# chongminggao/CIRS-codes

Hardware: AMD Instinct MI355X
Metric: simulator env-steps/s (collect + PPO update in the timed region), KuaishouEnv (higher is better)
Workload: dtype f32 (policy/tracker; rollout on the fp32 MFMA, PPO head products fp32-accurate from two fp16 pieces per operand (3 f16 MFMAs per product), fp32 accumulate) + f64 (env rewards, GAE)

## Files before the change

### cirs-codes_amd/csrc/ppo.hip

```cpp
#include "internal.h"
#include "bf16x6.h"
#include "small_gemm.h"
#include "permutation.h"
#include "policy_kernels.h"

namespace cirs {
typedef float f32x4 __attribute__((ext_vector_type(4)));


constexpr int kBwdWaves = 4;
__host__ __device__ inline int n_row_blocks_of(int n_pad) { return (n_pad / kTileM + kBwdWaves - 1) / kBwdWaves; }
__host__ __device__ inline size_t dwa_slab_stride(int I) { return (((size_t)I * 64 + I) + 3) & ~(size_t)3; }
__host__ __device__ inline int n_dwa_slabs_of(int n_pad) { return n_row_blocks_of(n_pad); }

struct PpoLayout {
    long w1, b1, w2, b2, wa, ba, wc, bc, total, trunk;
};
__host__ __device__ inline PpoLayout ppo_layout(int I, int S) {
    PpoLayout L;
    L.w1 = 0; L.b1 = L.w1 + (long)kH * S; L.w2 = L.b1 + kH; L.b2 = L.w2 + (long)kH * kH;
    L.trunk = L.b2 + kH;
    L.wa = L.trunk; L.ba = L.wa + (long)I * kH; L.wc = L.ba + I; L.bc = L.wc + kH; L.total = L.bc + 1;
    return L;
}
// ... 144 lines not shown
__global__ __launch_bounds__(1024) void prepare_tail_kernel(cirs_ppo_cfg cfg, cirs_traj traj, cirs_ppo_batch out, const double* __restrict__ unnorm_ret,
                                                            double* __restrict__ rms_state, const int32_t* __restrict__ n_dev, int B, int S, int n_compact,
                                                            PermKeys keys, int n_perm, long perm_upper, int32_t* __restrict__ perm_out) {
    __shared__ double red[1024];
    __shared__ double s_mean;
    const int N = *n_dev;
    const int b = blockIdx.x;
    if (b == 0) { returns_block(cfg, unnorm_ret, N, rms_state, out.ret, red, s_mean); return; }
    if (b <= n_compact) { compact_obs_elem(traj, out, (long)(b - 1) * 1024 + threadIdx.x, N, B, S); return; }
    const long g = (long)(b - 1 - n_compact) * 1024 + threadIdx.x;
    const int c = (int)(g / perm_upper);
    const long i = g - (long)c * perm_upper;
    if (c < n_perm && i < N) perm_out[(size_t)c * N + i] = (int32_t)permute_index(i, N, perm_half_bits((uint64_t)N), perm_key_of(keys, c));
}

typedef Planes2 HPl;
constexpr float kScWa = 256.f, kScH2 = 64.f;
#define HPL_SET(P, H, L) do { (P).h = __builtin_bit_cast(f16x8, H); (P).l = __builtin_bit_cast(f16x8, L); } while (0)
#define hsplit8 split8h
#define hmfma_split2 mfma_f16x3_split2
#define hmfma_pair mfma_f16x3_pair
constexpr float kScZ = kScWa * kScH2, kScZi = 1.0f / kScZ;
constexpr int kPlaneTileU4 = 1536;
struct MbView {
    float *obs, *adv, *ret, *v_s, *logp_old;
    int32_t* act;
    float *h1, *h2, *value;
    float *lse, *ez, *za;
    float *c_logp, *c_ent, *h_ent, *dvalue;
    float *ent_row;
    float *clip_row, *vf_row;
    long *dst_row;
    float *da2, *da1;
    float *dh2p;
    float *entp;
    float *dwap;
    float *red;
    float *normp;
    float *dwp;
    uint4 *wa_planes;
    uint4 *h2z, *h2b;
    int *sync;
    void* head_ws;
};

constexpr int kSyncInts = 288, kSyncA0 = 256;
__device__ __forceinline__ void flag_arrive(int* flags, int b) {
    if (threadIdx.x == 0) __hip_atomic_store(flags + b, 1, __ATOMIC_RELAXED, __HIP_MEMORY_SCOPE_AGENT);
}
__device__ int g_handoff_lost = 0;
__device__ __forceinline__ void flags_wait(const int* flags, int n) {
    int spins = 0;
    for (;;) {
        int mine = 1;
        for (int q = threadIdx.x; q < n; q += blockDim.x) mine &= __hip_atomic_load(flags + q, __ATOMIC_RELAXED, __HIP_MEMORY_SCOPE_AGENT) != 0;
        if (__syncthreads_and(mine)) break;
        if (++spins >= (1 << 20)) {
            if (threadIdx.x == 0) atomicAdd(&g_handoff_lost, 1);
            break;
        }
        __builtin_amdgcn_s_sleep(1);
    }
}
__global__ void handoff_status_kernel(int* __restrict__ out, int reset) {
    out[0] = g_handoff_lost;
// ... 13 lines not shown
__host__ __device__ inline int snap_floats(int S) { return kH * (S + 66) + kH + 1; }
__host__ __device__ inline int snap_stride(int S) { return (snap_floats(S) + 3) & ~3; }
__host__ inline size_t dwp_floats(int n_pad, int S) {
    const size_t a = (size_t)(n_pad / kTileM) * (kH * (kH + 1) + kH * (S + 1) + (kH + 1)) + 64, b = (size_t)(n_pad / 8) * snap_stride(S) + 64;
    return a > b ? a : b;
}
__host__ inline size_t mb_ws_floats(int n_pad, int I, int S) {
    const size_t nch = n_chunks_of(I);
    size_t f = 0;
    f += (size_t)n_pad * S + 4 * (size_t)n_pad;
    f += n_pad;
    f += 2 * (size_t)n_pad * kH + n_pad;
    f += 3 * (size_t)n_pad;
    f += 4 * (size_t)n_pad + n_pad;
    f += 2 * (size_t)n_pad + 2 * (size_t)n_pad + 8;
    f += 2 * (size_t)n_pad * kH;
    f += nch * (size_t)n_pad * kH + nch * (size_t)n_pad;
    f += (size_t)n_dwa_slabs_of(n_pad) * dwa_slab_stride(I);
    f += kSyncInts + 4;
    f += 64 + 1024;
    f += dwp_floats(n_pad, S);
    f += (size_t)cdiv(I, kTileN) * kPlaneTileU4 * 4;
    f += 2 * (size_t)n_pad * 96;
    f += (size_t)n_pad * kH + 4 * nch * (size_t)n_pad;
    return f;
}

__host__ inline MbView carve(void* ws, int n_pad, int I, int S) {
    float* p = (float*)ws;
    const size_t nch = n_chunks_of(I);
    MbView v;
    auto take = [&](size_t n) { float* r = p; p += (n + 3) & ~(size_t)3; return r; };
    v.obs = take((size_t)n_pad * S); v.adv = take(n_pad); v.ret = take(n_pad); v.v_s = take(n_pad); v.logp_old = take(n_pad);
    v.act = (int32_t*)take(n_pad);
    v.h1 = take((size_t)n_pad * kH); v.h2 = take((size_t)n_pad * kH); v.value = take(n_pad);
    v.lse = take(n_pad); v.ez = take(n_pad); v.za = take(n_pad);
    v.c_logp = take(n_pad); v.c_ent = take(n_pad); v.h_ent = take(n_pad); v.dvalue = take(n_pad); v.ent_row = take(n_pad);
    v.clip_row = take(n_pad); v.vf_row = take(n_pad);
    v.dst_row = (long*)take(2 * (size_t)n_pad + 4);
    v.da2 = take((size_t)n_pad * kH); v.da1 = take((size_t)n_pad * kH);
    v.dh2p = take(nch * (size_t)n_pad * kH); v.entp = take(nch * (size_t)n_pad);
    v.dwap = take((size_t)n_dwa_slabs_of(n_pad) * dwa_slab_stride(I));
    v.sync = (int*)take(kSyncInts);
    v.red = take(64);
    v.normp = take(1024);
    v.dwp = take(dwp_floats(n_pad, S));
    v.wa_planes = (uint4*)take((size_t)cdiv(I, kTileN) * kPlaneTileU4 * 4);
    v.h2z = (uint4*)take((size_t)n_pad * 96); v.h2b = (uint4*)take((size_t)n_pad * 96);
    v.head_ws = (void*)p;
    return v;
}

__device__ __forceinline__ void adv_stats_block(const float* __restrict__ adv_flat, const int32_t* __restrict__ idx, int m,
                                                int enable, float* __restrict__ red, float* sh ) {
    __shared__ float s_mean;
    const int tid = threadIdx.x;
    if (!enable) {
        if (tid == 0) { red[0] = 0.f; red[1] = 1.f; }
        return;
    }
    float acc = 0.f;
    for (int i = tid; i < m; i += 256) acc += adv_flat[idx[i]];
    sh[tid] = acc;
    __syncthreads();
    for (int s = 128; s > 0; s >>= 1) {
        if (tid < s) sh[tid] += sh[tid + s];
        __syncthreads();
    }
    if (tid == 0) s_mean = sh[0] / (float)m;
    __syncthreads();
    const float mean = s_mean;
// ... 259 lines not shown

constexpr int kTStride = 36;
constexpr int kRSize = kTileN * kH + 2 * kTileN;
constexpr int kRowB = 144, kColB = 80;
constexpr int kRPlaneB = kTileN * kRowB, kCPlaneB = kH * kColB;
constexpr int kWBufB = 3 * kRPlaneB + 3 * kCPlaneB;

#ifdef CIRS_HEAD_PROF
__device__ unsigned long long g_step_prof[64];
#define CIRS_PSTAMP(COND, K) do { if ((COND) && threadIdx.x == 0) g_step_prof[K] = __builtin_amdgcn_s_memtime(); } while (0)
#else
#define CIRS_PSTAMP(COND, K) do { } while (0)
#endif
#ifdef CIRS_HEAD_PROF
__device__ unsigned long long g_head_prof[64];
#define CIRS_HSTAMP(K) do { if (blockIdx.x == 0 && blockIdx.y == 0 && threadIdx.x == 0 && it == 2) g_head_prof[K] = __builtin_amdgcn_s_memtime(); } while (0)
#define CIRS_TSTAMP(B, K) do { if ((int)blockIdx.x == (B) && threadIdx.x == 0) g_head_prof[K] = __builtin_amdgcn_s_memtime(); } while (0)
#define CIRS_SSTAMP(K) do { if (blockIdx.x == 0 && blockIdx.y == 0 && threadIdx.x == 0) g_head_prof[K] = __builtin_amdgcn_s_memtime(); } while (0)
#else
#define CIRS_HSTAMP(K) do { } while (0)
#define CIRS_TSTAMP(B, K) do { } while (0)
#define CIRS_SSTAMP(K) do { } while (0)
#endif
__global__ __launch_bounds__(256, 2) void head_stats_kernel(int I, int mb, int n_pad, int tiles_per_chunk,
                                                            const uint4* __restrict__ planes, const float* __restrict__ ba,
                                                            const uint4* __restrict__ h2z, ActorPartialView pv,
                                                            const int32_t* __restrict__ act_rows, float* __restrict__ za_out) {
    __shared__ __attribute__((aligned(16))) unsigned char sW[2][3 * kRPlaneB];
    __shared__ __attribute__((aligned(16))) float sB[2][kTileN];
    const int tid = threadIdx.x;
    CIRS_SSTAMP(40);
    const int lane = tid & 63, wv = tid >> 6;
    const int hi = lane >> 5, lo = lane & 31;
    const int row0 = (blockIdx.y * 4 + wv) * kTileM;
    const int chunk = blockIdx.x;
    const int jr = row0 + lo;
    const bool wave_ok = row0 < n_pad && row0 < mb;
    const bool active = jr < mb;
    HPl hz[4];
    {
        const uint4* zp = h2z + (size_t)((wave_ok ? row0 : 0) >> 5) * 12 * 64 + lane;
#pragma unroll
        for (int s4 = 0; s4 < 4; ++s4) {
            HPL_SET(hz[s4], zp[(3 * s4) * 64], zp[(3 * s4 + 2) * 64]);
        }
    }
    float run_m = -INFINITY, run_s = 0.f, run_t = 0.f;
    const int act_r = (act_rows && active) ? act_rows[jr] : -1;
    float za_val = 0.f;
    bool za_have = false;
    const int first_tile = chunk * tiles_per_chunk * kTileN;
    const int n_tiles = max(0, min(tiles_per_chunk, (I - first_tile + kTileN - 1) / kTileN));
    const int dst_r = (tid >> 3) * kRowB + (tid & 7) * 16;
    uint4 g0, g2;
    float gb = 0.f;
#define CIRS_ISSUE(TILE0)                                                                                  \
    do {                                                                                                   \
        const uint4* src_ = planes + (size_t)((TILE0) / kTileN) * kPlaneTileU4 + tid;                      \
        g0 = src_[0]; g2 = src_[512];                                             \
        if (tid < kTileN) gb = ((TILE0) + tid) < I ? kScZ * ba[(TILE0) + tid] : 0.f;    \
// ... 10 lines not shown
    if (n_tiles > 0) { CIRS_ISSUE(first_tile); CIRS_COMMIT(0); }
    __syncthreads();
    CIRS_SSTAMP(42);
    for (int it = 0; it < n_tiles; ++it) {
        const int buf = it & 1;
        const int tile0 = first_tile + it * kTileN;
        if (it == 2) CIRS_SSTAMP(43);
        if (it + 1 < n_tiles) CIRS_ISSUE(tile0 + kTileN);
        if (wave_ok) {
            const unsigned char* tw = sW[buf];
            HPl za[4];
#pragma unroll
            for (int s4 = 0; s4 < 4; ++s4) {
                const unsigned char* ap = tw + lo * kRowB + (16 * s4 + 8 * hi) * 2;
                HPL_SET(za[s4], *reinterpret_cast<const uint4*>(ap), *reinterpret_cast<const uint4*>(ap + 2 * kRPlaneB));
            }
            f32x16 acc, accs, acct;
#pragma unroll
            for (int r = 0; r < 16; ++r) { acc[r] = sB[buf][acc_row(r, hi)]; accs[r] = 0.f; acct[r] = 0.f; }
            if (it == 2) CIRS_SSTAMP(44);
            hmfma_split2(za[0], hz[0], za[1], hz[1], acc, accs, acct);
            hmfma_split2(za[2], hz[2], za[3], hz[3], acc, accs, acct);
#pragma unroll
            for (int r = 0; r < 16; ++r) acc[r] = (acc[r] + (accs[r] + acct[r])) * kScZi;
            if (it == 2) CIRS_SSTAMP(45);
            {
                const int arel = act_r - tile0;
                const bool mine = act_r >= 0 && arel >= 0 && arel < kTileN && ((arel >> 2) & 1) == hi;
                if (__any(mine)) {
                    const int rsel = (arel & 3) + 4 * (arel >> 3);
                    float zsel = acc[0];
#pragma unroll
                    for (int r = 1; r < 16; ++r) zsel = rsel == r ? acc[r] : zsel;
                    if (mine) { za_val = zsel; za_have = true; }
                }
            }
            f32x16 zt = acc;
            if (tile0 + kTileN > I) {
#pragma unroll
                for (int r = 0; r < 16; ++r) zt[r] = tile0 + acc_row(r, hi) < I ? acc[r] : -INFINITY;
            }
            float tmax = zt[0];
#pragma unroll
            for (int r = 1; r < 16; ++r) tmax = fmaxf(tmax, zt[r]);
            if (tmax > -INFINITY) {
                const float mn = fmaxf(run_m, tmax);
                const float keep = __expf(run_m - mn);
// ... 20 lines not shown
    if (row0 >= n_pad) return;
    if (!active) { run_m = -INFINITY; run_s = 0.f; run_t = 0.f; }
    {
        const float om = __shfl_xor(run_m, 32, CIRS_WAVE), osum = __shfl_xor(run_s, 32, CIRS_WAVE);
        const float ot = __shfl_xor(run_t, 32, CIRS_WAVE);
        const float mn = fmaxf(run_m, om);
        if (mn > -INFINITY) {
            const float fa = __expf(run_m - mn), fb = __expf(om - mn);
            run_s = run_s * fa + osum * fb;
            run_t = run_t * fa + ot * fb;
            run_m = mn;
        }
    }
    if (hi == 0) {
        const size_t po = (size_t)chunk * n_pad + jr;
        pv.score[po] = run_t; pv.m[po] = run_m; pv.s[po] = run_s;
    }
    if (za_have) za_out[jr] = za_val;
}



struct HeadMergeArgs { cirs_ppo_cfg cfg; cirs_ppo_batch b; const int32_t* idx; int mb_norm, n_schunks; ActorPartialView pv; };
template <bool kEnt, bool kMerge>
__global__ __launch_bounds__(kBwdWaves * 64, 1) void head_bwd_fused_kernel(int I, int mb, int n_pad, int tiles_per_chunk,
                                                                         const uint4* __restrict__ planes,
                                                                         const float* __restrict__ ba, MbView v,
                                                                         float* __restrict__ dwap, HeadMergeArgs ma) {
    constexpr int kThreads = kBwdWaves * 64;
    static_assert(kThreads == 256, "the plane staging maps one 16-byte unit per thread and plane");
    __shared__ __attribute__((aligned(16))) unsigned char sW[2][kWBufB];
    __shared__ __attribute__((aligned(16))) float sB[2][kTileN];
    __shared__ __attribute__((aligned(16))) float sT[kBwdWaves][kTileN * kTStride];
    __shared__ __attribute__((aligned(16))) float sR[2][kBwdWaves][kRSize];
    const int tid = threadIdx.x;
    CIRS_SSTAMP(30);
    if (blockIdx.x == 0 && blockIdx.y == 0) {
        v.sync[tid] = 0;
        if (tid < kSyncInts - 256) v.sync[256 + tid] = 0;
    }
    const int lane = tid & 63, wv = tid >> 6;
    const int hi = lane >> 5, lo = lane & 31;
    const int row0 = (blockIdx.y * kBwdWaves + wv) * kTileM;
    const bool wave_ok = row0 < n_pad;
    const int chunk = blockIdx.x;
    if (chunk * tiles_per_chunk * kTileN >= I) return;
    const int jr = wave_ok ? row0 + lo : 0;
    const float kLog2e = 1.4426950408889634f, kLn2 = 0.6931471805599453f;
    const int act = v.act[jr];
    HPl hz[4];
    HPl hb[2][2];
    {
        const size_t tb = (size_t)((wave_ok ? row0 : 0) >> 5) * 12 * 64 + lane;
        const uint4* zp = v.h2z + tb;
        const uint4* bp = v.h2b + tb;
#pragma unroll
        for (int s4 = 0; s4 < 4; ++s4) {
            HPL_SET(hz[s4], zp[(3 * s4) * 64], zp[(3 * s4 + 2) * 64]);
        }
#pragma unroll
        for (int c = 0; c < 2; ++c)
#pragma unroll
            for (int t = 0; t < 2; ++t) {
                HPL_SET(hb[c][t], bp[(3 * (2 * c + t)) * 64], bp[(3 * (2 * c + t) + 2) * 64]);
            }
    }
    const bool row_ok = wave_ok && jr < mb;
    f32x16 dh0, dh1;
#pragma unroll
    for (int r = 0; r < 16; ++r) { dh0[r] = 0.f; dh1[r] = 0.f; }
    float ent = 0.f;
    const float eps = 1.1920928955078125e-7f;
    const float kLogEps = -15.942385152878742f, kLog1mEps = -1.1920929665620834e-7f;
    if (!wave_ok) {
        for (int q = lane; q < kRSize; q += 64) { sR[0][wv][q] = 0.f; sR[1][wv][q] = 0.f; }
    }

    const int first_tile = chunk * tiles_per_chunk * kTileN;
    const int n_tiles = max(0, min(tiles_per_chunk, (I - first_tile + kTileN - 1) / kTileN));
    const int dst_r = (tid >> 3) * kRowB + (tid & 7) * 16;
    const int dst_c = 3 * kRPlaneB + (tid >> 2) * kColB + (tid & 3) * 16;
    uint4 gr0, gr2, gc0, gc2;
    float gb = 0.f;
#define CIRS_ISSUE(TILE0)                                                                                  \
    do {                                                                                                   \
        const uint4* src_ = planes + (size_t)((TILE0) / kTileN) * kPlaneTileU4 + tid;                      \
        gr0 = src_[0]; gr2 = src_[512]; gc0 = src_[768]; gc2 = src_[1280]; \
        if (tid < kTileN) gb = ((TILE0) + tid) < I ? kScZ * ba[(TILE0) + tid] : 0.f;    \
    } while (0)
#define CIRS_COMMIT(BUF)                                                                                   \
    do {                                                                                                   \
        unsigned char* base_ = sW[BUF];                                                                    \
        *reinterpret_cast<uint4*>(base_ + dst_r) = gr0;                                                    \
        \
        *reinterpret_cast<uint4*>(base_ + 2 * kRPlaneB + dst_r) = gr2;                                     \
        *reinterpret_cast<uint4*>(base_ + dst_c) = gc0;                                                    \
        \
        *reinterpret_cast<uint4*>(base_ + 2 * kCPlaneB + dst_c) = gc2;                                     \
        if (tid < kTileN) sB[BUF][tid] = gb;                                                               \
    } while (0)
    if (n_tiles > 0) CIRS_ISSUE(first_tile);
    float lse, c_logp, c_ent, h_ent;
    if (!kMerge) {
        lse = v.lse[jr]; c_logp = v.c_logp[jr]; c_ent = kEnt ? v.c_ent[jr] : 0.f; h_ent = kEnt ? v.h_ent[jr] : 0.f;
    } else {
        const bool real = wave_ok && jr < mb;
        const int jc = real ? jr : 0;
        const float za = v.za[jc], adv = v.adv[jc], lpo = v.adv[n_pad + jc], ret = v.adv[2 * (size_t)n_pad + jc], vs = v.adv[3 * (size_t)n_pad + jc],
                    val = v.value[jc];
        const float red0 = v.red[0], red1 = v.red[1];
        const int nsc = ma.n_schunks;
        const float* __restrict__ pm_ = ma.pv.m + jc;
        const float* __restrict__ ps_ = ma.pv.s + jc;
        const float* __restrict__ pt_ = ma.pv.score + jc;
        float M = -INFINITY, ssum = 0.f, tsum = 0.f;
        const bool need_t = kEnt || blockIdx.x == 0;
        for (int cb = 0; cb < nsc; cb += 64) {
            const int c0 = cb + hi;
            float m32[32], s32[32], u32[32];
#pragma unroll
            for (int q = 0; q < 32; ++q) {
                const int c = c0 + 2 * q;
                const size_t o = (size_t)(c < nsc ? c : nsc - 1) * n_pad;
// ... 84 lines not shown
            if (full || t0 + (f >> 4) < I) *reinterpret_cast<f32x4*>(slab + (size_t)t0 * kH + 4 * f) = t;
        }
        if (wv == 0) {
            float t = rg.b[0];
#pragma unroll
            for (int w2 = 1; w2 < kBwdWaves; ++w2) t += rg.b[w2];
            if (hi == 0 && (full || t0 + lo < I)) slab[(size_t)I * kH + t0 + lo] = t * dz_inv;
        }
    };
    auto reduce_tile = [&](int rb, int t0) { RedRegs rg; reduce_load(rb, rg); reduce_store(rg, t0); };
    for (int it = 0; it < n_tiles; ++it) {
        const int buf = it & 1;
        const int tile0 = first_tile + it * kTileN;
        CIRS_HSTAMP(0);
        if (it + 1 < n_tiles) CIRS_ISSUE(tile0 + kTileN);
        f32x16 dw0, dw1;
        float db = 0.f;
        if (!wave_ok) {
            if (it + 1 < n_tiles) CIRS_COMMIT(buf ^ 1);
            if (it > 0) reduce_tile(buf ^ 1, tile0 - kTileN);
        }
        if (wave_ok) {
            const unsigned char* tw = sW[buf];
            HPl za[4], cb[2][2];
#pragma unroll
            for (int s4 = 0; s4 < 4; ++s4) {
                const unsigned char* ap = tw + lo * kRowB + (16 * s4 + 8 * hi) * 2;
                HPL_SET(za[s4], *reinterpret_cast<const uint4*>(ap), *reinterpret_cast<const uint4*>(ap + 2 * kRPlaneB));
            }
            f32x16 acc, acc1, acc2;
#pragma unroll
            for (int r = 0; r < 16; ++r) { acc[r] = sB[buf][acc_row(r, hi)]; acc1[r] = 0.f; acc2[r] = 0.f; }
            CIRS_HSTAMP(1);
            hmfma_split2(za[0], hz[0], za[1], hz[1], acc, acc1, acc2);
            RedRegs rg;
            if (it > 0) reduce_load(buf ^ 1, rg);
            hmfma_split2(za[2], hz[2], za[3], hz[3], acc, acc1, acc2);
#pragma unroll
            for (int r = 0; r < 16; ++r) acc1[r] += acc2[r];
            if (it > 0) reduce_store(rg, tile0 - kTileN);
#pragma unroll
            for (int t = 0; t < 2; ++t)
#pragma unroll
                for (int c = 0; c < 2; ++c) {
                    const unsigned char* bp = tw + 3 * kRPlaneB + (32 * c + lo) * kColB + (16 * t + 8 * hi) * 2;
                    HPL_SET(cb[c][t], *reinterpret_cast<const uint4*>(bp), *reinterpret_cast<const uint4*>(bp + 2 * kCPlaneB));
                }
            CIRS_HSTAMP(2);
            float* tt = sT[wv];
            f32x16 tk;
            float pmax = 0.f, elo = 0.f;
            f32x2_b elo2 = {0.f, 0.f};
            const float kTEps = -23.0f;
            const bool last_tile = tile0 + kTileN > I;
#pragma unroll
            for (int r = 0; r < 16; r += 2) {
                const float t0 = __builtin_fmaf(acc[r] + acc1[r], kLog2e * kScZi, nlse2), t1 = __builtin_fmaf(acc[r + 1] + acc1[r + 1], kLog2e * kScZi, nlse2);
                const float p0 = __builtin_amdgcn_exp2f(t0), p1 = __builtin_amdgcn_exp2f(t1);
                tk[r] = t0; tk[r + 1] = t1;
                pmax = __builtin_fmaxf(__builtin_fmaxf(pmax, p0), p1);
                if (!last_tile) {
                    const f32x2_b d2 = f32x2_b{kTEps, kTEps} - f32x2_b{t0, t1};
                    const f32x2_b w2 = {__builtin_fmaxf(d2.x, 0.f), __builtin_fmaxf(d2.y, 0.f)};
                    elo2 = f32x2_b{p0, p1} * w2 + elo2;
                }
                if (kEnt) {
                    acc[r] = __builtin_fmaf(c_ent * p0, __builtin_fmaf(t0, kLn2, h_ent), ncl * p0);
                    acc[r + 1] = __builtin_fmaf(c_ent * p1, __builtin_fmaf(t1, kLn2, h_ent), ncl * p1);
                } else {
                    acc[r] = ncl * p0; acc[r + 1] = ncl * p1;
                }
            }
            if (__any(act >= tile0 && act < tile0 + kTileN)) {
                const int rel = act - tile0 - 4 * hi;
#pragma unroll
                for (int r = 0; r < 16; ++r) acc[r] += (rel == (r & 3) + 8 * (r >> 2)) ? c_logp : 0.f;
            }
            if (last_tile) {
#pragma unroll
                for (int r = 0; r < 16; ++r) {
// ... 7 lines not shown
#pragma unroll
            for (int r = 0; r < 16; ++r) tt[acc_row(r, hi) * kTStride + lo] = acc[r];
            if (__any(row_ok && pmax > 1.0f - eps)) {
#pragma unroll
                for (int r = 0; r < 16; ++r) {
                    const float p = __builtin_amdgcn_exp2f(tk[r]);
                    const bool ok = row_ok && (!last_tile || tile0 + acc_row(r, hi) < I);
                    ent -= (ok && p > 1.0f - eps) ? p * (kLog1mEps - tk[r] * kLn2) : 0.f;
                }
            }
            CIRS_HSTAMP(4);
            __builtin_amdgcn_fence(__ATOMIC_RELEASE, "wavefront");
            __builtin_amdgcn_wave_barrier();
            __builtin_amdgcn_fence(__ATOMIC_ACQUIRE, "wavefront");
            f32x16 dzt;
#pragma unroll
            for (int g = 0; g < 4; ++g) {
                const float4 t4 = *reinterpret_cast<const float4*>(&tt[lo * kTStride + 8 * g + 4 * hi]);
                dzt[4 * g] = t4.x; dzt[4 * g + 1] = t4.y; dzt[4 * g + 2] = t4.z; dzt[4 * g + 3] = t4.w;
            }
            if (it + 1 < n_tiles) CIRS_COMMIT(buf ^ 1);
            {
                const HPl a0 = hsplit8(acc, 0), a1 = hsplit8(acc, 8);
                hmfma_pair(a0, cb[0][0], cb[1][0], dh0, dh1);
                hmfma_pair(a1, cb[0][1], cb[1][1], dh0, dh1);
            }
            CIRS_HSTAMP(5);
            CIRS_HSTAMP(6);
#pragma unroll
            for (int r = 0; r < 16; ++r) { dw0[r] = 0.f; dw1[r] = 0.f; db += dzt[r]; }
            {
                const HPl b0 = hsplit8(dzt, 0), b1 = hsplit8(dzt, 8);
                hmfma_pair(b0, hb[0][0], hb[1][0], dw0, dw1);
                hmfma_pair(b1, hb[0][1], hb[1][1], dw0, dw1);
            }
        }
        CIRS_HSTAMP(7);
        if (wave_ok) {
            float* rr = sR[buf][wv];
#pragma unroll
            for (int r = 0; r < 16; ++r) {
                const int il = acc_row(r, hi);
                rr[il * kH + lo] = dw0[r];
                rr[il * kH + 32 + lo] = dw1[r];
            }
            rr[kTileN * kH + lane] = db;
        }
        CIRS_HSTAMP(9);
        lds_barrier();
        CIRS_HSTAMP(10);
    }
    CIRS_SSTAMP(33);
    if (n_tiles > 0) reduce_tile((n_tiles - 1) & 1, first_tile + (n_tiles - 1) * kTileN);
    CIRS_SSTAMP(34);
#undef CIRS_ISSUE
#undef CIRS_COMMIT
    if (!wave_ok) return;
    float* hslab = v.dh2p + (size_t)chunk * n_pad * kH;
#pragma unroll
    for (int r = 0; r < 16; ++r) {
        const int row = row0 + acc_row(r, hi);
        hslab[(size_t)row * kH + lo] = dh0[r] * dh_unscale;
        hslab[(size_t)row * kH + 32 + lo] = dh1[r] * dh_unscale;
    }
    ent += __shfl_xor(ent, 32, CIRS_WAVE);
    if (hi == 0) v.entp[(size_t)chunk * n_pad + jr] = ent;
    CIRS_SSTAMP(35);
}

constexpr int kNormBlocks = 256;
constexpr int kWaSumBlocks = 176;
__device__ __forceinline__ void wa_slab_sum_block(float* __restrict__ g, long wa_beg, long wa_len, const float* __restrict__ dwap,
                                                  long slab_stride, int n_slabs, int b, float* __restrict__ partial_out, float* sh) {
    const int tid = threadIdx.x;
    float acc = 0.f;
    const long n4 = wa_len >> 2;
    for (long q4 = b * 1024L + tid; q4 < n4; q4 += (long)kWaSumBlocks * 1024) {
        const long q4b = q4 + 512;
        const bool has_b = q4b < n4;
        f32x4 ta[8], tb[8];
#pragma unroll
        for (int q = 0; q < 8; ++q) {
            ta[q] = q < n_slabs ? *reinterpret_cast<const f32x4*>(dwap + (size_t)q * slab_stride + 4 * q4) : f32x4{0.f, 0.f, 0.f, 0.f};
            tb[q] = (has_b && q < n_slabs) ? *reinterpret_cast<const f32x4*>(dwap + (size_t)q * slab_stride + 4 * q4b) : f32x4{0.f, 0.f, 0.f, 0.f};
        }
        f32x4 x = {0.f, 0.f, 0.f, 0.f}, y = {0.f, 0.f, 0.f, 0.f};
#pragma unroll
        for (int q = 0; q < 8; ++q) { x += ta[q]; y += tb[q]; }
        for (int s0 = 8; s0 < n_slabs; ++s0) {
            x += *reinterpret_cast<const f32x4*>(dwap + (size_t)s0 * slab_stride + 4 * q4);
// ... 1198 lines not shown
extern "C" int cirs_adam_step(float* params, const float* grads, float* m, float* v, int64_t n, int64_t step_before,
                              int32_t n_sub, float lr, float beta1, float beta2, float eps, const float* grad_scale,
                              int32_t scale_pow, void* stream) {
    using namespace cirs;
    CIRS_REQUIRE(params && grads && m && v && n > 0, "bad arguments");
    return launch_adam(params, grads, m, v, n, step_before, n_sub, lr, beta1, beta2, eps, grad_scale, scale_pow, (hipStream_t)stream);
}

struct PpoRun {
    const cirs_ppo_cfg* cfg;
    float *params, *grads, *adam_m, *adam_v;
    const cirs_ppo_batch* batch;
    int n_env;
    void* workspace;
    int n_pad_carve;
    hipStream_t s;
    int I, S;
    cirs::PpoLayout L;
    cirs_policy_cfg pcfg;
    cirs_policy_weights w;
    cirs::MbView v;
    float* tail;
    bool merge_launch;
};
struct PpoStep { const int32_t* idx; int mb; const int32_t* sidx; int mb_norm; float* dobs; float* loss_out; long opt_step; };

static PpoRun ppo_run(const cirs_ppo_cfg* cfg, float* params, float* grads, float* adam_m, float* adam_v, const cirs_ppo_batch* batch, int n_env,
                      void* workspace, int max_mb, hipStream_t s) {
    using namespace cirs;
    PpoRun r;
    r.cfg = cfg; r.params = params; r.grads = grads; r.adam_m = adam_m; r.adam_v = adam_v; r.batch = batch; r.n_env = n_env; r.workspace = workspace;
    r.n_pad_carve = n_pad_of(max_mb); r.s = s; r.I = cfg->n_items; r.S = cfg->dim_state;
    r.L = ppo_layout(r.I, r.S);
    r.pcfg = cirs_policy_cfg{r.I, r.S, kH};
    r.w = cirs_policy_weights{params + r.L.w1, params + r.L.b1, params + r.L.w2, params + r.L.b2, params + r.L.wa, params + r.L.ba, params + r.L.wc,
                              params + r.L.bc};
    r.v = carve(workspace, r.n_pad_carve, r.I, r.S);
    r.tail = grads + r.L.total;
    const char* mk_ = getenv("CIRS_PPO_MERGE_KERNEL");
    r.merge_launch = mk_ && atoi(mk_) != 0;
    return r;
}
static cirs::TrunkRowOut trunk_out_of(const cirs::MbView& v) { return cirs::TrunkRowOut{v.h2, v.value, v.h1, v.obs, v.act, v.dst_row, v.adv, v.h2z, v.h2b}; }

static int launch_trunk_adv(const PpoRun& r, const PpoStep& st) {
    using namespace cirs;
    const int n_pad = n_pad_of(st.mb);
    hipLaunchKernelGGL(trunk_adv_kernel, dim3(cdiv(n_pad, 4) + 1 + cdiv(r.I, kTileN)), dim3(256), 0, r.s, r.pcfg, r.w, (const float*)r.batch->obs, (long)r.S,
                       n_pad, st.idx, st.mb, (const float*)r.batch->adv, st.sidx, st.mb_norm, (int)r.cfg->norm_adv, r.v.red, (int)cdiv(n_pad, 4),
                       r.v.wa_planes, *r.batch, r.n_env, trunk_out_of(r.v));
    CIRS_CHECK_LAUNCH("trunk_adv_kernel");
    return CIRS_OK;
}
static int launch_head(const PpoRun& r, const PpoStep& st, int* n_bchunks_out, bool with_dh2_sum) {
    using namespace cirs;
    const int I = r.I, mb = st.mb, n_pad = n_pad_of(mb), n_slabs = n_row_blocks_of(n_pad);
    const MbView& v = r.v;
    ActorPartialView pv = partial_view(v.head_ws, n_pad, I);
    const int n_item_tiles = cdiv(I, kTileN);
    const int tpc_s = head_tiles_per_chunk(n_item_tiles, n_slabs, 2);
    const int n_schunks = cdiv(n_item_tiles, tpc_s);
    CIRS_PROF_LAUNCH(2, r.s, hipLaunchKernelGGL(head_stats_kernel, dim3(n_schunks, n_slabs), dim3(256), 0, r.s, I, mb, n_pad, tpc_s,
                                                (const uint4*)v.wa_planes, r.w.ba, (const uint4*)v.h2z, pv, (const int32_t*)v.act, v.za));
    CIRS_CHECK_LAUNCH("head_stats_kernel");
    const HeadMergeArgs hma{*r.cfg, *r.batch, st.idx, st.mb_norm, n_schunks, pv};
    if (r.merge_launch) {
        hipLaunchKernelGGL(head_stats_merge_kernel, dim3(cdiv(n_pad, 4)), dim3(256), 0, r.s, *r.cfg, *r.batch, st.idx, mb, st.mb_norm, n_pad, n_schunks,
                           r.n_env, pv, r.w.wa, r.w.ba, v, (const float*)nullptr, 0);
        CIRS_CHECK_LAUNCH("head_stats_merge_kernel");
    }
    const int tpc = head_tiles_per_chunk(n_item_tiles, n_slabs, 1);
    const int n_bchunks = cdiv(n_item_tiles, tpc);
    const dim3 bgrid((n_bchunks + 7) & ~7, n_slabs), bblock(kBwdWaves * 64);
    if (r.cfg->ent_coef != 0.f) {
        if (r.merge_launch) CIRS_PROF_LAUNCH(1, r.s, hipLaunchKernelGGL((head_bwd_fused_kernel<true, false>), bgrid, bblock, 0, r.s, I, mb, n_pad, tpc, (const uint4*)v.wa_planes, r.w.ba, v, v.dwap, hma));
        else CIRS_PROF_LAUNCH(1, r.s, hipLaunchKernelGGL((head_bwd_fused_kernel<true, true>), bgrid, bblock, 0, r.s, I, mb, n_pad, tpc, (const uint4*)v.wa_planes, r.w.ba, v, v.dwap, hma));
    } else {
        if (r.merge_launch) CIRS_PROF_LAUNCH(1, r.s, hipLaunchKernelGGL((head_bwd_fused_kernel<false, false>), bgrid, bblock, 0, r.s, I, mb, n_pad, tpc, (const uint4*)v.wa_planes, r.w.ba, v, v.dwap, hma));
        else CIRS_PROF_LAUNCH(1, r.s, hipLaunchKernelGGL((head_bwd_fused_kernel<false, true>), bgrid, bblock, 0, r.s, I, mb, n_pad, tpc, (const uint4*)v.wa_planes, r.w.ba, v, v.dwap, hma));
    }
    CIRS_CHECK_LAUNCH("head_bwd_fused_kernel");
    if (with_dh2_sum) {
        hipLaunchKernelGGL(dh2_sum_kernel, dim3(n_pad * (kH / 4) / 64 + cdiv(n_pad, 64)), dim3(64), 0, r.s, mb, n_pad, n_bchunks, v);
        CIRS_CHECK_LAUNCH("dh2_sum_kernel");
    }
    *n_bchunks_out = n_bchunks;
    return CIRS_OK;
}
static cirs::DwJobs trunk_dw_jobs(const PpoRun& r, int n_pad) {
    using namespace cirs;
    const MbView& v = r.v;
    DwJobs jobs{};
    jobs.n = 3;
    jobs.j[0] = DwJob{v.dvalue, 1, v.h2, kH, 1, kH, r.grads + r.L.wc, r.grads + r.L.bc, 0, 0};
    jobs.j[1] = DwJob{v.da2, kH, v.h1, kH, kH, kH, r.grads + r.L.w2, r.grads + r.L.b2, 0, 0};
    jobs.j[2] = DwJob{v.da1, kH, v.obs, r.S, kH, r.S, r.grads + r.L.w1, r.grads + r.L.b1, 0, 0};
    const int n_dw_slabs = n_pad / kTileM;
    int off = 0, out = 0;
    for (int q = 0; q < 3; ++q) {
        jobs.j[q].part_off = off;
        off += n_dw_slabs * jobs.j[q].O * (jobs.j[q].K + 1);
        out += jobs.j[q].O * (jobs.j[q].K + 1);
    }
// ... 257 lines not shown
    const int I = cfg->n_items, S = cfg->dim_state;
    CIRS_REQUIRE(S <= 32, "dim_state > 32 is not supported by the trunk backward kernel");
    const int n_pad = n_pad_of(mb);
    const PpoLayout L = ppo_layout(I, S);
    MbView v = carve(workspace, n_pad, I, S);
    cirs_policy_cfg pcfg{I, S, kH};
    cirs_policy_weights w{params + L.w1, params + L.b1, params + L.w2, params + L.b2, params + L.wa, params + L.ba, params + L.wc, params + L.bc};
    const long seg = (long)I * kH + I;
    const int n_slabs = n_row_blocks_of(n_pad);
    const int n_item_tiles = cdiv(I, kTileN);
    float* red_dh2 = red;
    float* red_ent = red + (size_t)n_pad * kH;
    float* red_slots = red_ent + n_pad;
    float* tail = grads + L.total;
    if (phase == 1) {
        CIRS_REQUIRE(stats4, "stats4 is null");
        hipLaunchKernelGGL(trunk_adv_kernel, dim3(cdiv(n_pad, 4) + 1 + cdiv(I, kTileN)), dim3(256), 0, s, pcfg, w, (const float*)batch->obs, (long)S, n_pad,
                           idx, (int)mb, (const float*)batch->adv, idx, (int)mb, (int)cfg->norm_adv, v.red, (int)cdiv(n_pad, 4), v.wa_planes, *batch, (int)n_env,
                           TrunkRowOut{v.h2, v.value, v.h1, v.obs, nullptr, nullptr, nullptr, v.h2z, v.h2b});
        CIRS_CHECK_LAUNCH("trunk_adv_kernel");
        ActorPartialView pv = partial_view(v.head_ws, n_pad, I);
        const int tpc_s = head_tiles_per_chunk(n_item_tiles, n_slabs, 2);
        const int n_schunks = cdiv(n_item_tiles, tpc_s);
        hipLaunchKernelGGL(head_stats_kernel, dim3(n_schunks, n_slabs), dim3(256), 0, s, I, (int)mb, n_pad, tpc_s, (const uint4*)v.wa_planes, w.ba,
                           (const uint4*)v.h2z, pv, (const int32_t*)nullptr, (float*)nullptr);
        CIRS_CHECK_LAUNCH("head_stats_kernel");
        hipLaunchKernelGGL(head_tp_fold_kernel, dim3(cdiv(n_pad, 4)), dim3(256), 0, s, *batch, idx, (int)mb, n_pad, n_schunks, pv, (const float*)w.wa,
                           (const float*)w.ba, (int)item_base, I, (const float*)v.h2, stats4);
        CIRS_CHECK_LAUNCH("head_tp_fold_kernel");
        return CIRS_OK;
    }
    if (phase == 2) {
        CIRS_REQUIRE(stats_all, "stats_all is null");
        ActorPartialView pa;
        pa.m = const_cast<float*>(stats_all); pa.s = pa.m + (size_t)world * n_pad; pa.score = pa.s + (size_t)world * n_pad;
        pa.idx = nullptr; pa.z = nullptr;
        const float* za = pa.score + (size_t)world * n_pad;
        hipLaunchKernelGGL(head_stats_merge_kernel, dim3(cdiv(n_pad, 4)), dim3(256), 0, s, *cfg, *batch, idx, (int)mb, (int)mb, n_pad, (int)world,
                           (int)n_env, pa, (const float*)nullptr, (const float*)nullptr, v, za, (int)item_base);
        CIRS_CHECK_LAUNCH("head_stats_merge_kernel");
        const int tpc = head_tiles_per_chunk(n_item_tiles, n_slabs, 1);
        const int n_bchunks = cdiv(n_item_tiles, tpc);
        const HeadMergeArgs no_merge{};
        if (cfg->ent_coef != 0.f) {
            hipLaunchKernelGGL((head_bwd_fused_kernel<true, false>), dim3((n_bchunks + 7) & ~7, n_slabs), dim3(kBwdWaves * 64), 0, s, I, mb, n_pad, tpc,
                               (const uint4*)v.wa_planes, w.ba, v, v.dwap, no_merge);
        } else {
            hipLaunchKernelGGL((head_bwd_fused_kernel<false, false>), dim3((n_bchunks + 7) & ~7, n_slabs), dim3(kBwdWaves * 64), 0, s, I, mb, n_pad, tpc,
                               (const uint4*)v.wa_planes, w.ba, v, v.dwap, no_merge);
        }
        CIRS_CHECK_LAUNCH("head_bwd_fused_kernel");
        CIRS_HIP(hipMemsetAsync(red_slots, 0, sizeof(float) * (size_t)world * kWaSumBlocks, s));
        hipLaunchKernelGGL(dh2_sum_kernel, dim3(n_pad * (kH / 4) / 64 + cdiv(n_pad, 64)), dim3(64), 0, s, (int)mb, n_pad, n_bchunks, v, red_dh2, red_ent);
        CIRS_CHECK_LAUNCH("dh2_sum_kernel");
        hipLaunchKernelGGL(wa_slab_sum_kernel, dim3(kWaSumBlocks), dim3(512), 0, s, grads, (long)L.wa, seg, (const float*)v.dwap,
                           (long)dwa_slab_stride(I), n_slabs, red_slots + (size_t)rank * kWaSumBlocks);
        CIRS_CHECK_LAUNCH("wa_slab_sum_kernel");
        return CIRS_OK;
    }
    CIRS_REQUIRE(loss_out, "loss_out is null");
    hipLaunchKernelGGL(tp_post_kernel, dim3(cdiv(n_pad, 256)), dim3(256), 0, s, (int)mb, n_pad, (int)world, (const float*)red_ent,
                       (const float*)red_slots, v);
    CIRS_CHECK_LAUNCH("tp_post_kernel");
    DwJobs jobs;
    jobs.n = 3;
    jobs.j[0] = DwJob{v.dvalue, 1, v.h2, kH, 1, kH, grads + L.wc, grads + L.bc, 0, 0};
    jobs.j[1] = DwJob{v.da2, kH, v.h1, kH, kH, kH, grads + L.w2, grads + L.b2, 0, 0};
    jobs.j[2] = DwJob{v.da1, kH, v.obs, S, kH, S, grads + L.w1, grads + L.b1, 0, 0};
    const int n_dw_slabs = n_pad / kTileM;
    {
        int off = 0, out = 0;
        for (int q = 0; q < 3; ++q) {
            jobs.j[q].part_off = off;
// ... 51 lines not shown
```

Before: 5.395 million.

## Store head logits from stats pass and reuse them in backward instead of recomputing

The stats kernel now writes the unscaled split-fp16 logit tiles (acc before the kScZi scale) into a new z-slab workspace. The fused backward kernel reads those tiles with a one-tile prefetch instead of staging the Wa row planes and bias and redoing the 3-MFMA split products. This removes the backward logit GEMM and about half its plane staging and LDS use. In exchange it adds a global write and read of an item-by-row fp32 slab. The old recompute path stays available behind an environment variable.

```diff
diff --git a/cirs-codes_amd/csrc/ppo.hip b/cirs-codes_amd/csrc/ppo.hip
--- a/cirs-codes_amd/csrc/ppo.hip
+++ b/cirs-codes_amd/csrc/ppo.hip
@@ -190,6 +190,8 @@
 #define hmfma_pair mfma_f16x3_pair
 constexpr float kScZ = kScWa * kScH2, kScZi = 1.0f / kScZ;
 constexpr int kPlaneTileU4 = 1536;
+constexpr int kZTileF4 = 256;
+__host__ inline size_t zslab_floats(int n_pad, int I) { return (size_t)cdiv(I, kTileN) * (n_pad / kTileM) * (kZTileF4 * 4); }
 struct MbView {
     float *obs, *adv, *ret, *v_s, *logp_old;
     int32_t* act;
@@ -209,6 +211,7 @@
     uint4 *wa_planes;
     uint4 *h2z, *h2b;
     int *sync;
+    float4 *zslab;
     void* head_ws;
 };
 
@@ -268,6 +271,7 @@
     f += dwp_floats(n_pad, S);
     f += (size_t)cdiv(I, kTileN) * kPlaneTileU4 * 4;
     f += 2 * (size_t)n_pad * 96;
+    f += zslab_floats(n_pad, I);
     f += (size_t)n_pad * kH + 4 * nch * (size_t)n_pad;
     return f;
 }
@@ -293,6 +297,7 @@
     v.dwp = take(dwp_floats(n_pad, S));
     v.wa_planes = (uint4*)take((size_t)cdiv(I, kTileN) * kPlaneTileU4 * 4);
     v.h2z = (uint4*)take((size_t)n_pad * 96); v.h2b = (uint4*)take((size_t)n_pad * 96);
+    v.zslab = (float4*)take(zslab_floats(n_pad, I));
     v.head_ws = (void*)p;
     return v;
 }
@@ -598,10 +603,12 @@
 #define CIRS_TSTAMP(B, K) do { } while (0)
 #define CIRS_SSTAMP(K) do { } while (0)
 #endif
+template <bool kZout>
 __global__ __launch_bounds__(256, 2) void head_stats_kernel(int I, int mb, int n_pad, int tiles_per_chunk,
                                                             const uint4* __restrict__ planes, const float* __restrict__ ba,
                                                             const uint4* __restrict__ h2z, ActorPartialView pv,
-                                                            const int32_t* __restrict__ act_rows, float* __restrict__ za_out) {
+                                                            const int32_t* __restrict__ act_rows, float* __restrict__ za_out,
+                                                            float4* __restrict__ zslab) {
     __shared__ __attribute__((aligned(16))) unsigned char sW[2][3 * kRPlaneB];
     __shared__ __attribute__((aligned(16))) float sB[2][kTileN];
     const int tid = threadIdx.x;
@@ -611,7 +618,7 @@
     const int row0 = (blockIdx.y * 4 + wv) * kTileM;
     const int chunk = blockIdx.x;
     const int jr = row0 + lo;
-    const bool wave_ok = row0 < n_pad && row0 < mb;
+    const bool wave_ok = row0 < n_pad && (kZout || row0 < mb);
     const bool active = jr < mb;
     HPl hz[4];
     {
@@ -668,7 +675,14 @@
             hmfma_split2(za[0], hz[0], za[1], hz[1], acc, accs, acct);
             hmfma_split2(za[2], hz[2], za[3], hz[3], acc, accs, acct);
 #pragma unroll
-            for (int r = 0; r < 16; ++r) acc[r] = (acc[r] + (accs[r] + acct[r])) * kScZi;
+            for (int r = 0; r < 16; ++r) acc[r] = acc[r] + (accs[r] + acct[r]);
+            if (kZout) {
+                float4* zp = zslab + ((size_t)(tile0 / kTileN) * (n_pad / kTileM) + (row0 / kTileM)) * kZTileF4 + lane;
+#pragma unroll
+                for (int q = 0; q < 4; ++q) zp[q * 64] = float4{acc[4 * q], acc[4 * q + 1], acc[4 * q + 2], acc[4 * q + 3]};
+            }
+#pragma unroll
+            for (int r = 0; r < 16; ++r) acc[r] *= kScZi;
             if (it == 2) CIRS_SSTAMP(45);
             {
                 const int arel = act_r - tile0;
@@ -735,14 +749,15 @@
 
 
 struct HeadMergeArgs { cirs_ppo_cfg cfg; cirs_ppo_batch b; const int32_t* idx; int mb_norm, n_schunks; ActorPartialView pv; };
-template <bool kEnt, bool kMerge>
+template <bool kEnt, bool kMerge, bool kZin>
 __global__ __launch_bounds__(kBwdWaves * 64, 1) void head_bwd_fused_kernel(int I, int mb, int n_pad, int tiles_per_chunk,
                                                                          const uint4* __restrict__ planes,
                                                                          const float* __restrict__ ba, MbView v,
                                                                          float* __restrict__ dwap, HeadMergeArgs ma) {
     constexpr int kThreads = kBwdWaves * 64;
     static_assert(kThreads == 256, "the plane staging maps one 16-byte unit per thread and plane");
-    __shared__ __attribute__((aligned(16))) unsigned char sW[2][kWBufB];
+    constexpr int kCOff = kZin ? 0 : 3 * kRPlaneB;
+    __shared__ __attribute__((aligned(16))) unsigned char sW[2][kCOff + 3 * kCPlaneB];
     __shared__ __attribute__((aligned(16))) float sB[2][kTileN];
     __shared__ __attribute__((aligned(16))) float sT[kBwdWaves][kTileN * kTStride];
     __shared__ __attribute__((aligned(16))) float sR[2][kBwdWaves][kRSize];
@@ -767,9 +782,11 @@
         const size_t tb = (size_t)((wave_ok ? row0 : 0) >> 5) * 12 * 64 + lane;
         const uint4* zp = v.h2z + tb;
         const uint4* bp = v.h2b + tb;
-#pragma unroll
-        for (int s4 = 0; s4 < 4; ++s4) {
-            HPL_SET(hz[s4], zp[(3 * s4) * 64], zp[(3 * s4 + 2) * 64]);
+        if (!kZin) {
+#pragma unroll
+            for (int s4 = 0; s4 < 4; ++s4) {
+                HPL_SET(hz[s4], zp[(3 * s4) * 64], zp[(3 * s4 + 2) * 64]);
+            }
         }
 #pragma unroll
         for (int c = 0; c < 2; ++c)
@@ -792,26 +809,35 @@
     const int first_tile = chunk * tiles_per_chunk * kTileN;
     const int n_tiles = max(0, min(tiles_per_chunk, (I - first_tile + kTileN - 1) / kTileN));
     const int dst_r = (tid >> 3) * kRowB + (tid & 7) * 16;
-    const int dst_c = 3 * kRPlaneB + (tid >> 2) * kColB + (tid & 3) * 16;
+    const int dst_c = kCOff + (tid >> 2) * kColB + (tid & 3) * 16;
     uint4 gr0, gr2, gc0, gc2;
     float gb = 0.f;
 #define CIRS_ISSUE(TILE0)                                                                                  \
     do {                                                                                                   \
         const uint4* src_ = planes + (size_t)((TILE0) / kTileN) * kPlaneTileU4 + tid;                      \
-        gr0 = src_[0]; gr2 = src_[512]; gc0 = src_[768]; gc2 = src_[1280]; \
-        if (tid < kTileN) gb = ((TILE0) + tid) < I ? kScZ * ba[(TILE0) + tid] : 0.f;    \
+        if (!kZin) { gr0 = src_[0]; gr2 = src_[512]; }                                                     \
+        gc0 = src_[768]; gc2 = src_[1280];                                                                 \
+        if (!kZin && tid < kTileN) gb = ((TILE0) + tid) < I ? kScZ * ba[(TILE0) + tid] : 0.f;    \
     } while (0)
 #define CIRS_COMMIT(BUF)                                                                                   \
     do {                                                                                                   \
         unsigned char* base_ = sW[BUF];                                                                    \
-        *reinterpret_cast<uint4*>(base_ + dst_r) = gr0;                                                    \
-        \
-        *reinterpret_cast<uint4*>(base_ + 2 * kRPlaneB + dst_r) = gr2;                                     \
+        if (!kZin) {                                                                                       \
+            *reinterpret_cast<uint4*>(base_ + dst_r) = gr0;                                                \
+            *reinterpret_cast<uint4*>(base_ + 2 * kRPlaneB + dst_r) = gr2;                                 \
+        }                                                                                                  \
         *reinterpret_cast<uint4*>(base_ + dst_c) = gc0;                                                    \
         \
         *reinterpret_cast<uint4*>(base_ + 2 * kCPlaneB + dst_c) = gc2;                                     \
-        if (tid < kTileN) sB[BUF][tid] = gb;                                                               \
+        if (!kZin && tid < kTileN) sB[BUF][tid] = gb;                                                      \
     } while (0)
+    const float4* zsl = v.zslab + ((size_t)(first_tile / kTileN) * (n_pad / kTileM) + (wave_ok ? row0 / kTileM : 0)) * kZTileF4 + lane;
+    const size_t zstep = (size_t)(n_pad / kTileM) * kZTileF4;
+    float4 zn[4];
+    if (kZin) {
+#pragma unroll
+        for (int q = 0; q < 4; ++q) zn[q] = zsl[q * 64];
+    }
     if (n_tiles > 0) CIRS_ISSUE(first_tile);
     float lse, c_logp, c_ent, h_ent;
     if (!kMerge) {
@@ -942,28 +968,39 @@
         }
         if (wave_ok) {
             const unsigned char* tw = sW[buf];
-            HPl za[4], cb[2][2];
-#pragma unroll
-            for (int s4 = 0; s4 < 4; ++s4) {
-                const unsigned char* ap = tw + lo * kRowB + (16 * s4 + 8 * hi) * 2;
-                HPL_SET(za[s4], *reinterpret_cast<const uint4*>(ap), *reinterpret_cast<const uint4*>(ap + 2 * kRPlaneB));
+            HPl cb[2][2];
+            f32x16 acc;
+            RedRegs rg;
+            if (kZin) {
+#pragma unroll
+                for (int q = 0; q < 4; ++q) { acc[4 * q] = zn[q].x; acc[4 * q + 1] = zn[q].y; acc[4 * q + 2] = zn[q].z; acc[4 * q + 3] = zn[q].w; }
+                const float4* zp = zsl + (size_t)min(it + 1, n_tiles - 1) * zstep;
+#pragma unroll
+                for (int q = 0; q < 4; ++q) zn[q] = zp[q * 64];
+                CIRS_HSTAMP(1);
+            } else {
+                HPl za[4];
+#pragma unroll
+                for (int s4 = 0; s4 < 4; ++s4) {
+                    const unsigned char* ap = tw + lo * kRowB + (16 * s4 + 8 * hi) * 2;
+                    HPL_SET(za[s4], *reinterpret_cast<const uint4*>(ap), *reinterpret_cast<const uint4*>(ap + 2 * kRPlaneB));
+                }
+                f32x16 acc1, acc2;
+#pragma unroll
+                for (int r = 0; r < 16; ++r) { acc[r] = sB[buf][acc_row(r, hi)]; acc1[r] = 0.f; acc2[r] = 0.f; }
+                CIRS_HSTAMP(1);
+                hmfma_split2(za[0], hz[0], za[1], hz[1], acc, acc1, acc2);
+                if (it > 0) reduce_load(buf ^ 1, rg);
+                hmfma_split2(za[2], hz[2], za[3], hz[3], acc, acc1, acc2);
+#pragma unroll
+                for (int r = 0; r < 16; ++r) acc[r] += acc1[r] + acc2[r];
+                if (it > 0) reduce_store(rg, tile0 - kTileN);
             }
-            f32x16 acc, acc1, acc2;
-#pragma unroll
-            for (int r = 0; r < 16; ++r) { acc[r] = sB[buf][acc_row(r, hi)]; acc1[r] = 0.f; acc2[r] = 0.f; }
-            CIRS_HSTAMP(1);
-            hmfma_split2(za[0], hz[0], za[1], hz[1], acc, acc1, acc2);
-            RedRegs rg;
-            if (it > 0) reduce_load(buf ^ 1, rg);
-            hmfma_split2(za[2], hz[2], za[3], hz[3], acc, acc1, acc2);
-#pragma unroll
-            for (int r = 0; r < 16; ++r) acc1[r] += acc2[r];
-            if (it > 0) reduce_store(rg, tile0 - kTileN);
 #pragma unroll
             for (int t = 0; t < 2; ++t)
 #pragma unroll
                 for (int c = 0; c < 2; ++c) {
-                    const unsigned char* bp = tw + 3 * kRPlaneB + (32 * c + lo) * kColB + (16 * t + 8 * hi) * 2;
+                    const unsigned char* bp = tw + kCOff + (32 * c + lo) * kColB + (16 * t + 8 * hi) * 2;
                     HPL_SET(cb[c][t], *reinterpret_cast<const uint4*>(bp), *reinterpret_cast<const uint4*>(bp + 2 * kCPlaneB));
                 }
             CIRS_HSTAMP(2);
@@ -975,7 +1012,7 @@
             const bool last_tile = tile0 + kTileN > I;
 #pragma unroll
             for (int r = 0; r < 16; r += 2) {
-                const float t0 = __builtin_fmaf(acc[r] + acc1[r], kLog2e * kScZi, nlse2), t1 = __builtin_fmaf(acc[r + 1] + acc1[r + 1], kLog2e * kScZi, nlse2);
+                const float t0 = __builtin_fmaf(acc[r], kLog2e * kScZi, nlse2), t1 = __builtin_fmaf(acc[r + 1], kLog2e * kScZi, nlse2);
                 const float p0 = __builtin_amdgcn_exp2f(t0), p1 = __builtin_amdgcn_exp2f(t1);
                 tk[r] = t0; tk[r + 1] = t1;
                 pmax = __builtin_fmaxf(__builtin_fmaxf(pmax, p0), p1);
@@ -1029,8 +1066,10 @@
             if (it + 1 < n_tiles) CIRS_COMMIT(buf ^ 1);
             {
                 const HPl a0 = hsplit8(acc, 0), a1 = hsplit8(acc, 8);
+                if (kZin && it > 0) reduce_load(buf ^ 1, rg);
                 hmfma_pair(a0, cb[0][0], cb[1][0], dh0, dh1);
                 hmfma_pair(a1, cb[0][1], cb[1][1], dh0, dh1);
+                if (kZin && it > 0) reduce_store(rg, tile0 - kTileN);
             }
             CIRS_HSTAMP(5);
             CIRS_HSTAMP(6);
@@ -1073,6 +1112,23 @@
     ent += __shfl_xor(ent, 32, CIRS_WAVE);
     if (hi == 0) v.entp[(size_t)chunk * n_pad + jr] = ent;
     CIRS_SSTAMP(35);
+}
+typedef void (*HeadBwdFn)(int, int, int, int, const uint4*, const float*, MbView, float*, HeadMergeArgs);
+__host__ inline HeadBwdFn head_bwd_fn(bool ent, bool merge, bool zin) {
+    switch ((ent ? 4 : 0) | (merge ? 2 : 0) | (zin ? 1 : 0)) {
+    case 0: return head_bwd_fused_kernel<false, false, false>;
+    case 1: return head_bwd_fused_kernel<false, false, true>;
+    case 2: return head_bwd_fused_kernel<false, true, false>;
+    case 3: return head_bwd_fused_kernel<false, true, true>;
+    case 4: return head_bwd_fused_kernel<true, false, false>;
+    case 5: return head_bwd_fused_kernel<true, false, true>;
+    case 6: return head_bwd_fused_kernel<true, true, false>;
+    default: return head_bwd_fused_kernel<true, true, true>;
+    }
+}
+__host__ inline bool head_recompute_env() {
+    const char* e = getenv("CIRS_PPO_HEAD_RECOMPUTE");
+    return e && atoi(e) != 0;
 }
 
 constexpr int kNormBlocks = 256;
@@ -2317,6 +2373,7 @@
     cirs::MbView v;
     float* tail;
     bool merge_launch;
+    bool head_recompute;
 };
 struct PpoStep { const int32_t* idx; int mb; const int32_t* sidx; int mb_norm; float* dobs; float* loss_out; long opt_step; };
 
@@ -2334,6 +2391,7 @@
     r.tail = grads + r.L.total;
     const char* mk_ = getenv("CIRS_PPO_MERGE_KERNEL");
     r.merge_launch = mk_ && atoi(mk_) != 0;
+    r.head_recompute = head_recompute_env();
     return r;
 }
 static cirs::TrunkRowOut trunk_out_of(const cirs::MbView& v) { return cirs::TrunkRowOut{v.h2, v.value, v.h1, v.obs, v.act, v.dst_row, v.adv, v.h2z, v.h2b}; }
@@ -2355,8 +2413,9 @@
     const int n_item_tiles = cdiv(I, kTileN);
     const int tpc_s = head_tiles_per_chunk(n_item_tiles, n_slabs, 2);
     const int n_schunks = cdiv(n_item_tiles, tpc_s);
-    CIRS_PROF_LAUNCH(2, r.s, hipLaunchKernelGGL(head_stats_kernel, dim3(n_schunks, n_slabs), dim3(256), 0, r.s, I, mb, n_pad, tpc_s,
-                                                (const uint4*)v.wa_planes, r.w.ba, (const uint4*)v.h2z, pv, (const int32_t*)v.act, v.za));
+    const auto stats_fn = r.head_recompute ? head_stats_kernel<false> : head_stats_kernel<true>;
+    CIRS_PROF_LAUNCH(2, r.s, hipLaunchKernelGGL(stats_fn, dim3(n_schunks, n_slabs), dim3(256), 0, r.s, I, mb, n_pad, tpc_s,
+                                                (const uint4*)v.wa_planes, r.w.ba, (const uint4*)v.h2z, pv, (const int32_t*)v.act, v.za, v.zslab));
     CIRS_CHECK_LAUNCH("head_stats_kernel");
     const HeadMergeArgs hma{*r.cfg, *r.batch, st.idx, st.mb_norm, n_schunks, pv};
     if (r.merge_launch) {
@@ -2367,13 +2426,8 @@
     const int tpc = head_tiles_per_chunk(n_item_tiles, n_slabs, 1);
     const int n_bchunks = cdiv(n_item_tiles, tpc);
     const dim3 bgrid((n_bchunks + 7) & ~7, n_slabs), bblock(kBwdWaves * 64);
-    if (r.cfg->ent_coef != 0.f) {
-        if (r.merge_launch) CIRS_PROF_LAUNCH(1, r.s, hipLaunchKernelGGL((head_bwd_fused_kernel<true, false>), bgrid, bblock, 0, r.s, I, mb, n_pad, tpc, (const uint4*)v.wa_planes, r.w.ba, v, v.dwap, hma));
-        else CIRS_PROF_LAUNCH(1, r.s, hipLaunchKernelGGL((head_bwd_fused_kernel<true, true>), bgrid, bblock, 0, r.s, I, mb, n_pad, tpc, (const uint4*)v.wa_planes, r.w.ba, v, v.dwap, hma));
-    } else {
-        if (r.merge_launch) CIRS_PROF_LAUNCH(1, r.s, hipLaunchKernelGGL((head_bwd_fused_kernel<false, false>), bgrid, bblock, 0, r.s, I, mb, n_pad, tpc, (const uint4*)v.wa_planes, r.w.ba, v, v.dwap, hma));
-        else CIRS_PROF_LAUNCH(1, r.s, hipLaunchKernelGGL((head_bwd_fused_kernel<false, true>), bgrid, bblock, 0, r.s, I, mb, n_pad, tpc, (const uint4*)v.wa_planes, r.w.ba, v, v.dwap, hma));
-    }
+    const HeadBwdFn bwd_fn = head_bwd_fn(r.cfg->ent_coef != 0.f, !r.merge_launch, !r.head_recompute);
+    CIRS_PROF_LAUNCH(1, r.s, hipLaunchKernelGGL(bwd_fn, bgrid, bblock, 0, r.s, I, mb, n_pad, tpc, (const uint4*)v.wa_planes, (const float*)r.w.ba, v, v.dwap, hma));
     CIRS_CHECK_LAUNCH("head_bwd_fused_kernel");
     if (with_dh2_sum) {
         hipLaunchKernelGGL(dh2_sum_kernel, dim3(n_pad * (kH / 4) / 64 + cdiv(n_pad, 64)), dim3(64), 0, r.s, mb, n_pad, n_bchunks, v);
@@ -2677,8 +2731,9 @@
         ActorPartialView pv = partial_view(v.head_ws, n_pad, I);
         const int tpc_s = head_tiles_per_chunk(n_item_tiles, n_slabs, 2);
         const int n_schunks = cdiv(n_item_tiles, tpc_s);
-        hipLaunchKernelGGL(head_stats_kernel, dim3(n_schunks, n_slabs), dim3(256), 0, s, I, (int)mb, n_pad, tpc_s, (const uint4*)v.wa_planes, w.ba,
-                           (const uint4*)v.h2z, pv, (const int32_t*)nullptr, (float*)nullptr);
+        const auto stats_fn = head_recompute_env() ? head_stats_kernel<false> : head_stats_kernel<true>;
+        hipLaunchKernelGGL(stats_fn, dim3(n_schunks, n_slabs), dim3(256), 0, s, I, (int)mb, n_pad, tpc_s, (const uint4*)v.wa_planes, (const float*)w.ba,
+                           (const uint4*)v.h2z, pv, (const int32_t*)nullptr, (float*)nullptr, v.zslab);
         CIRS_CHECK_LAUNCH("head_stats_kernel");
         hipLaunchKernelGGL(head_tp_fold_kernel, dim3(cdiv(n_pad, 4)), dim3(256), 0, s, *batch, idx, (int)mb, n_pad, n_schunks, pv, (const float*)w.wa,
                            (const float*)w.ba, (int)item_base, I, (const float*)v.h2, stats4);
@@ -2697,13 +2752,8 @@
         const int tpc = head_tiles_per_chunk(n_item_tiles, n_slabs, 1);
         const int n_bchunks = cdiv(n_item_tiles, tpc);
         const HeadMergeArgs no_merge{};
-        if (cfg->ent_coef != 0.f) {
-            hipLaunchKernelGGL((head_bwd_fused_kernel<true, false>), dim3((n_bchunks + 7) & ~7, n_slabs), dim3(kBwdWaves * 64), 0, s, I, mb, n_pad, tpc,
-                               (const uint4*)v.wa_planes, w.ba, v, v.dwap, no_merge);
-        } else {
-            hipLaunchKernelGGL((head_bwd_fused_kernel<false, false>), dim3((n_bchunks + 7) & ~7, n_slabs), dim3(kBwdWaves * 64), 0, s, I, mb, n_pad, tpc,
-                               (const uint4*)v.wa_planes, w.ba, v, v.dwap, no_merge);
-        }
+        hipLaunchKernelGGL(head_bwd_fn(cfg->ent_coef != 0.f, false, !head_recompute_env()), dim3((n_bchunks + 7) & ~7, n_slabs), dim3(kBwdWaves * 64), 0, s, I,
+                           (int)mb, n_pad, tpc, (const uint4*)v.wa_planes, (const float*)w.ba, v, v.dwap, no_merge);
         CIRS_CHECK_LAUNCH("head_bwd_fused_kernel");
         CIRS_HIP(hipMemsetAsync(red_slots, 0, sizeof(float) * (size_t)world * kWaSumBlocks, s));
         hipLaunchKernelGGL(dh2_sum_kernel, dim3(n_pad * (kH / 4) / 64 + cdiv(n_pad, 64)), dim3(64), 0, s, (int)mb, n_pad, n_bchunks, v, red_dh2, red_ent);
```

After: 5.552 million (median of 6 runs). 1.03x the previous value.
